# Triton-AI/Triton-Racer-Sim

Hardware: AMD Instinct MI355X
Metric: env-steps/s (whole node) at N envs x 120x160 RGB (higher is better)
Workload: dtype f32 state / f64 nearest-point / u8 image; 1 GPU; 1024 envs/GPU x 1 GPU, bicycle physics + L1 nearest point + 120x160 RGB pinhole rasteriser = BASELINE configs[2], generated_track 1185 pts, synthetic controls seed 0x5EED, auto-reset; envs_total=1024, envs_per_gpu=1024, img_h=120, img_w=160, depth=False, steps_per_launch=1, step_mode=resident worker (posted steps), prewarm_steps=8400, launcher=self

## Files before the change

### triton-racer-sim_amd/csrc/trsim_device.hpp

```cpp
#pragma once
#include <hip/hip_runtime.h>

#include <cstdint>

#include "../../include/trsim.h"
#include "../../include/trsim_spec.h"
#include "trsim_plan.hpp"
#include "trsim_tables.hpp"

#ifndef TRS_ABLATE
#define TRS_ABLATE 0
#endif

namespace trsim {

struct PParams {
    float *x, *y, *z, *yaw, *v, *speed, *cte, *ep_return, *last_return, *steer_filt;
    int32_t *seg_idx, *ep_len;
    uint8_t *done, *pending;
    const float *ctl_steer, *ctl_thr, *ctl_brk;
    const uint8_t* ctl_reset;
    int ctl_stride;
    float4* cam;
    const unsigned char* blob;
// ... 403 lines not shown
    o.is_done = is_done; o.do_reset = do_reset;
}

template <bool SEL = false>
__device__ __forceinline__ void env_step(const PParams& p, const unsigned char* lphys, int e, EnvRegs& s, uint32_t t, int k,
                                         float4* cam_out, float4* lcam_slot, int* pprog_j, int lane, const trsim::HillBlock* hill = nullptr, float* lpitch_slot = nullptr)
{
    const uint8_t rin = (!p.synth && p.ctl_reset && k == 0) ? p.ctl_reset[e] : (uint8_t)0;
    float steer = 0.f, thr = 0.f, brk = 0.f;
    if (!p.synth) {
        const size_t ci = (size_t)k * (size_t)p.ctl_stride + (size_t)e;
        steer = p.ctl_steer[ci]; thr = p.ctl_thr[ci]; brk = p.ctl_brk ? p.ctl_brk[ci] : 0.0f;
    }
    StepOut o;
    env_advance<false, true, SEL>(p, lphys, e, s, t, p.synth, steer, thr, brk, rin, lane, o, hill);
    if (lane == 0) {
        if (p.write_cam) cam_out[e] = o.cam;
        *lcam_slot = o.cam;
        if (hill) {
            if (p.write_cam) hill->cam_pitch[(size_t)(t & (kRing - 1)) * p.n_envs + e] = o.pitch;
            if (lpitch_slot) *lpitch_slot = o.pitch;
        }
        if (o.is_done) atomicAdd(&p.stats[0], 1ull);
        if (o.do_reset) atomicAdd(&p.stats[1], 1ull);
        __hip_atomic_store(pprog_j, k + 1, __ATOMIC_RELEASE, __HIP_MEMORY_SCOPE_WORKGROUP);
    }
}

__device__ __forceinline__ f2v ray_step(f2v kk2, f2v cns)
{
#ifdef TRS_PACKED_RAY_STEP
    return kk2 * cns;
#else
    float dx, dz;
    asm("v_mul_f32 %0, %1, %2" : "=v"(dx) : "v"(kk2.x), "v"(cns.x));
    asm("v_mul_f32 %0, %1, %2" : "=v"(dz) : "v"(kk2.y), "v"(cns.y));
    return f2v{dx, dz};
#endif
}

struct RasterThread {
    const f2v* lrow;
    const float* lrowdepth;
    unsigned pal_off;
    f2v ufa, ufb, ufc, ufd;
    unsigned gwm1, ghm1, pitch;
    int cg, vstart, vground, col_off, row_bytes;
};

__device__ __forceinline__ RasterThread raster_thread(const RParams& p, const unsigned char* lds, int tid)
{
    RasterThread t;
    t.lrow = reinterpret_cast<const f2v*>(lds + p.off_rowtab);
    t.lrowdepth = reinterpret_cast<const float*>(lds + p.off_depth);
    t.pal_off = (unsigned)p.off_pal;
    const float half_w = (float)(p.W / 2);
    t.gwm1 = (unsigned)(p.map_w - 1); t.ghm1 = (unsigned)(p.map_h - 1);
    t.cg = tid % p.gpr;
    const int r0 = tid / p.gpr;
    const float uf0 = (float)(t.cg << 2) + 0.5f - half_w;
    t.ufa = f2v{uf0, uf0}; t.ufb = f2v{uf0 + 1.0f, uf0 + 1.0f}; t.ufc = f2v{uf0 + 2.0f, uf0 + 2.0f}; t.ufd = f2v{uf0 + 3.0f, uf0 + 3.0f};
    t.pitch = (unsigned)p.map_pitch_b;
    t.vstart = r0 < p.rows_per_pass ? r0 : p.H;
    t.vground = t.vstart;
    while (t.vground < p.uni_rows) t.vground += p.rows_per_pass;
    t.row_bytes = p.gpr * 12;
    t.col_off = t.cg * 12;
    return t;
}

struct FrameDesc { __amdgpu_buffer_rsrc_t rgb, dep; };

template <bool DEPTH>
__device__ __forceinline__ FrameDesc frame_desc(const RParams& p, uint8_t* img, float* dep, int e)
{
    FrameDesc f;
    f.rgb = __builtin_amdgcn_make_buffer_rsrc(img + (size_t)e * ((size_t)p.gpe * 12), 0, (int)((size_t)p.gpe * 12), 0x00020000);
    f.dep = f.rgb;
    if constexpr (DEPTH) f.dep = __builtin_amdgcn_make_buffer_rsrc(dep + (size_t)e * ((size_t)p.gpe * 4), 0, (int)((size_t)p.gpe * 16), 0x00020000);
    return f;
}

template <bool DEPTH>
__device__ __forceinline__ void raster_uniform_rows(const RParams& p, const RasterThread& t, const FrameDesc& f, int uni_rows = -1)
{
    const int nu = uni_rows < 0 ? p.uni_rows : uni_rows;
    for (int v = t.vstart; v < nu; v += p.rows_per_pass) {
        const uint32_t c = *(lds_u32p)(uintptr_t)(t.pal_off + ((unsigned)v << 4));
        const u3v px3 = {__builtin_amdgcn_perm(c, c, 0x04020100u), __builtin_amdgcn_perm(c, c, 0x05040201u), __builtin_amdgcn_perm(c, c, 0x06050402u)};
        __builtin_amdgcn_raw_buffer_store_b96(px3, f.rgb, t.col_off + v * t.row_bytes, 0, TRS_STORE_AUX);
        if constexpr (DEPTH) {
            const unsigned dz = __float_as_uint(t.lrowdepth[v]);
            const u4v d4 = {dz, dz, dz, dz};
            __builtin_amdgcn_raw_buffer_store_b128(d4, f.dep, (t.cg + v * p.gpr) * 16, 0, TRS_STORE_AUX);
        }
    }
}

template <bool DEPTH, bool UNI_CHECK = false>
__device__ __forceinline__ void raster_ground_rows(const RParams& p, const RasterThread& t, const FrameDesc& f, const float4 cam)
{
    const f2v sc = {cam.z, cam.w}, cns = {cam.w, -cam.z}, camxz = {cam.x, cam.y};
    f2v rt = t.lrow[t.vground < p.H ? t.vground : 0];
    for (int v = t.vground; v < p.H; v += p.rows_per_pass) {
        const int vn = v + p.rows_per_pass;
        const f2v rtn = t.lrow[vn < p.H ? vn : v];
        const unsigned pal_a = t.pal_off + ((unsigned)v << 4);
        const f2v lz2 = {rt.x, rt.x}, kk2 = {rt.y, rt.y};
        f2v a;
        if constexpr (UNI_CHECK) {
            a.x = __builtin_fmaf(rt.x, sc.x, camxz.x);
            a.y = __builtin_fmaf(rt.x, sc.y, camxz.y);
        } else {
            a = __builtin_elementwise_fma(lz2, sc, camxz);
        }
        const f2v d = ray_step(kk2, cns);
        auto shade = [&](f2v uf) -> uint32_t {
            const f2v g = __builtin_elementwise_fma(uf, d, a);
            const unsigned ix = min(cvt_u32_sat(g.x), t.gwm1);
            const unsigned iz = min(cvt_u32_sat(g.y), t.ghm1);
            const unsigned xoff = (ix >> 2) & ~3u;
            unsigned waddr, paddr;
            asm("v_mad_u32_u24 %0, %1, %2, %3" : "=v"(waddr) : "v"(iz), "s"(t.pitch), "v"(xoff));
            const uint32_t w = *(lds_u32p)(uintptr_t)waddr;
            const uint32_t cls = __builtin_amdgcn_ubfe(w, ix << 1, 2);
            asm("v_lshl_add_u32 %0, %1, 2, %2" : "=v"(paddr) : "v"(cls), "v"(pal_a));
            return *(lds_u32p)(uintptr_t)paddr;
        };
#if TRS_ABLATE == 2
        const uint32_t c0p = (uint32_t)v, c1p = c0p + 1, c2p = c0p + 2, c3p = c0p + 3; (void)shade;
#else
        uint32_t c0p, c1p, c2p, c3p;
        if (UNI_CHECK && rt.y == 0.0f) c0p = c1p = c2p = c3p = *(lds_u32p)(uintptr_t)pal_a;
        else { c0p = shade(t.ufa); c1p = shade(t.ufb); c2p = shade(t.ufc); c3p = shade(t.ufd); }
#endif
        const uint32_t w0 = __builtin_amdgcn_perm(c1p, c0p, 0x04020100u);
        const uint32_t w1 = __builtin_amdgcn_perm(c2p, c1p, 0x05040201u);
        const uint32_t w2 = __builtin_amdgcn_perm(c3p, c2p, 0x06050402u);
#if TRS_ABLATE == 1
        asm volatile("" :: "v"(w0), "v"(w1), "v"(w2)); (void)f;
#else
        const u3v px3 = {w0, w1, w2};
        __builtin_amdgcn_raw_buffer_store_b96(px3, f.rgb, t.col_off + v * t.row_bytes, 0, TRS_STORE_AUX);
        if constexpr (DEPTH) {
            const unsigned dz = __float_as_uint(t.lrowdepth[v]);
            const u4v d4 = {dz, dz, dz, dz};
            __builtin_amdgcn_raw_buffer_store_b128(d4, f.dep, (t.cg + v * p.gpr) * 16, 0, TRS_STORE_AUX);
        }
#endif
        rt = rtn;
    }
}


__device__ __forceinline__ uint32_t hill_filter_colour(const trsim::HillBlock& hb, uint32_t bgr)
{
    int t[3];
#pragma unroll
    for (int ch = 0; ch < 3; ++ch) {
        float x = (float)((bgr >> (8 * ch)) & 255u);
        x = x - hb.f_offset;
        x = x * hb.f_contrast;
        x = x + hb.f_offset;
        x = x < 0.0f ? 0.0f : (x > 255.0f ? 255.0f : x);
        t[ch] = (int)x;
    }
    int o0 = t[0], o1 = t[1], o2 = t[2];
    if (hb.f_color) {
        const int r = t[0], g = t[1], b = t[2];
        const int vv = max(r, max(g, b)), vmin = min(r, min(g, b)), diff = vv - vmin;
        const int sat = (diff * hb.hsv_tab[vv] + (1 << 11)) >> 12;
        int h = (vv == r) ? (g - b) : ((vv == g) ? (b - r + 2 * diff) : (r - g + 4 * diff));
        h = (h * hb.hsv_tab[256 + diff] + (1 << 11)) >> 12;
        if (h < 0) h += 180;
        const int hh = min(h, 255), ss = min(sat, 255);
#pragma unroll
        for (int f = 0; f < 4; ++f) {
            if (f >= hb.f_nfilters) break;
            const int lo = (int)hb.f_lo[f], hi = (int)hb.f_hi[f];
            const bool in = hh >= (lo & 255) && hh <= (hi & 255) && ss >= ((lo >> 8) & 255) && ss <= ((hi >> 8) & 255) && vv >= ((lo >> 16) & 255) && vv <= ((hi >> 16) & 255);
            const int val = in ? 255 : 0, d = hb.f_dst[f];
            o0 = d == 0 ? val : o0; o1 = d == 1 ? val : o1; o2 = d == 2 ? val : o2;
        }
    }
    return (uint32_t)o0 | ((uint32_t)o1 << 8) | ((uint32_t)o2 << 16);
}

__device__ __forceinline__ float hill_row_build(const RParams& p, unsigned char* lds, unsigned tab_off, float P, int v, const float* lg = nullptr)
{
    const trsim::HillBlock hb = *hill_block(p);
    float sp, cp;
    spec_sincos(P, sp, cp);
    const float yn = (hb.hh - ((float)v + 0.5f)) * hb.inv_f;
    const float dy = yn * cp - sp, dz = yn * sp + cp;
    float lz = 0.0f, kk = 0.0f, dep = hb.z_far_f;
    uint32_t c0, c1, c2, c3;
    if (dy >= -1e-6f) {
        c0 = c1 = c2 = c3 = *(lds_u32p)(uintptr_t)((unsigned)hb.off_sky + ((unsigned)v << 2));
        if (lg) { c0 = trsim::light_colour(c0, lg); if (hb.filt) c0 = hill_filter_colour(hb, c0); c1 = c2 = c3 = c0; }
    } else {
        const float t = hb.cam_h_f / (-dy);
        const float zd = t * dz;
        if (zd > hb.z_far_f) {
            c0 = c1 = c2 = c3 = hb.far_rgb;
            if (lg) { c0 = trsim::light_colour(c0, lg); if (hb.filt) c0 = hill_filter_colour(hb, c0); c1 = c2 = c3 = c0; }
        } else {
            lz = zd * hb.inv_cell_f; kk = (t * hb.inv_f) * hb.inv_cell_f; dep = zd;
            const float fw = hb.fog_f * (zd * hb.inv_zfar_f), om = 1.0f - fw;
            constexpr int base[4][3] = {TRS_RGB_GRASS, TRS_RGB_ROAD, TRS_RGB_EDGE, TRS_RGB_CENTRE};
            constexpr int fog[3] = TRS_RGB_FOG;
            uint32_t col[4];
#pragma unroll
            for (int c = 0; c < 4; ++c) {
                uint32_t rgb = 0;
#pragma unroll
                for (int ch = 0; ch < 3; ++ch) {
                    const float a = (float)base[c][ch] * om, b = (float)fog[ch] * fw;
                    const float sum = a + b;
                    rgb |= (uint32_t)(int)(sum + 0.5f) << (8 * ch);
                }
                if (lg) rgb = trsim::light_colour(rgb, lg);
                col[c] = hb.filt ? hill_filter_colour(hb, rgb) : rgb;
            }
            c0 = col[0]; c1 = col[1]; c2 = col[2]; c3 = col[3];
        }
    }
    unsigned char* const tab = lds + tab_off;
    reinterpret_cast<f2v*>(tab)[v] = f2v{lz, kk};
    reinterpret_cast<u4v*>(tab + trsim::hill_table_pal_off(p.H))[v] = u4v{c0, c1, c2, c3};
    reinterpret_cast<float*>(tab + trsim::hill_table_depth_off(p.H))[v] = dep;
    return kk;
}

__device__ __forceinline__ RasterThread raster_use_table(const RasterThread& t, const unsigned char* lds, unsigned tab_off, int H)
{
    RasterThread r = t;
    r.lrow = reinterpret_cast<const f2v*>(lds + tab_off);
    r.pal_off = tab_off + (unsigned)trsim::hill_table_pal_off(H);
    r.lrowdepth = reinterpret_cast<const float*>(lds + tab_off + (unsigned)trsim::hill_table_depth_off(H));
    return r;
}

template <typename Bail>
__device__ __forceinline__ bool team_barrier_wait(const int* dbar, int target, Bail& bail)
{
    for (unsigned spins = 0; __hip_atomic_load(dbar, __ATOMIC_ACQUIRE, __HIP_MEMORY_SCOPE_WORKGROUP) < target; ++spins) {
        __builtin_amdgcn_s_sleep(1);
        if ((spins & 1023u) == 1023u && bail(spins == 1023u)) return false;
    }
    return true;
}

template <typename Bail>
__device__ __forceinline__ bool hill_batch_build(const RParams& p, unsigned char* lds, unsigned tab0, const float (&P)[kHillBatchMax], int nb, int* hbar, int done_before,
                                                 int tid, int lane, Bail& bail, const float* lg0 = nullptr)
{
    constexpr int nrw = kRasterThreads / 64;
    int* const fg = hbar + 4 + 4 * ((done_before / (2 * nrw)) & 1);
    if (tid < kHillBatchMax) fg[tid] = p.H;
    asm volatile("s_waitcnt lgkmcnt(0)" ::: "memory");
    if (lane == 0) __hip_atomic_fetch_add(hbar, 1, __ATOMIC_RELEASE, __HIP_MEMORY_SCOPE_WORKGROUP);
    if (!team_barrier_wait(hbar, done_before + nrw, bail)) return false;
    const unsigned tb = (unsigned)hill_table_bytes(p.H);
    for (int row = tid; row < nb * p.H; row += kRasterThreads) {
        const int bi = row / p.H, v = row - bi * p.H;
        const float Pv = bi == 0 ? P[0] : (bi == 1 ? P[1] : (bi == 2 ? P[2] : P[3]));
        if (hill_row_build(p, lds, tab0 + (unsigned)bi * tb, Pv, v, lg0 ? lg0 + 8 * bi : nullptr) != 0.0f) __hip_atomic_fetch_min(&fg[bi], v, __ATOMIC_RELAXED, __HIP_MEMORY_SCOPE_WORKGROUP);
    }
    asm volatile("s_waitcnt lgkmcnt(0)" ::: "memory");
    if (lane == 0) __hip_atomic_fetch_add(hbar, 1, __ATOMIC_RELEASE, __HIP_MEMORY_SCOPE_WORKGROUP);
    return team_barrier_wait(hbar, done_before + 2 * nrw, bail);
}

template <bool DEPTH>
__device__ __forceinline__ void raster_hill_frame(const RParams& p, const RasterThread& rth, const unsigned char* lds, unsigned tab0, int bi, const int* hbar, int done_before,
                                                  const FrameDesc& f, const float4 cam)
{
    constexpr int nrw = kRasterThreads / 64;
    const int first_ground = hbar[4 + 4 * ((done_before / (2 * nrw)) & 1) + bi];
    RasterThread t = raster_use_table(rth, lds, tab0 + (unsigned)(bi * hill_table_bytes(p.H)), p.H);
    raster_uniform_rows<DEPTH>(p, t, f, first_ground);
    int vg = t.vstart;
    if (vg < first_ground) vg += ((first_ground - vg + p.rows_per_pass - 1) / p.rows_per_pass) * p.rows_per_pass;
    t.vground = vg;
    raster_ground_rows<DEPTH, true>(p, t, f, cam);
}

__device__ __forceinline__ unsigned light_wave_palette(const RParams& p, unsigned pal0, const float* lg, int filt, int wave, int lane)
{
    const unsigned dst = pal0 + (unsigned)((wave % light_copies(p.gpr)) * p.H * 16);
    const int lo = (64 * wave) / p.gpr, hi = min((64 * wave + 63) / p.gpr, p.rows_per_pass - 1);
    const trsim::HillBlock& hb = *hill_block(p);
    float gb[8];
#pragma unroll
    for (int k = 0; k < 8; ++k) gb[k] = lg[k];
    asm volatile("" ::: "memory");
    for (int r0 = lo; r0 <= hi; ++r0)
        for (int i = lane; r0 + (i >> 2) * p.rows_per_pass < p.H; i += 64) {
            const unsigned ent = ((unsigned)(r0 + (i >> 2) * p.rows_per_pass) << 4) + ((unsigned)(i & 3) << 2);
            uint32_t c = trsim::light_colour(*(lds_u32p)(uintptr_t)((unsigned)p.off_pal + ent), gb);
            if (filt) c = hill_filter_colour(hb, c);
            *(__attribute__((address_space(3))) uint32_t*)(uintptr_t)(dst + ent) = c;
        }
    asm volatile("" ::: "memory");
    return dst;
}
// ... 451 lines not shown
```

### triton-racer-sim_amd/csrc/trsim_resident.hip

```cpp
#include <hip/hip_runtime.h>

#include <algorithm>
#include <array>
#include <atomic>
#include <chrono>
#include <cstdint>
#include <cstdlib>
#include <cstring>
#include <mutex>
#include <string>
#include <utility>

#include "../../include/trsim.h"
#include "../../include/trsim_spec.h"
#include "trsim_device.hpp"
#include "trsim_env.hpp"
#include "trsim_internal.hpp"
#include "trsim_post.hpp"

namespace trsim {

struct DevCtl {
    alignas(64) unsigned long long word;
    alignas(64) WEntry ring[kSlots];
// ... 330 lines not shown
        }
    }
}

template <bool DEPTH, bool DYN, bool HILLS = false, bool LENS = false, bool LIGHT = false>
__global__ __launch_bounds__(kBlock) void trs_worker_kernel(const WParams wp)
{
    const int tid = threadIdx.x, lane = tid & 63, wave = tid >> 6;
    const bool raster_team = tid < kRasterThreads;
    const RParams& p = wp.ra;
    const PParams& P = wp.ph;
    const int epw = p.envs_per_wg;
    const WLds l = wlds_of(smem + wp.lds_off_ctl, epw);
    const int e_begin = blockIdx.x * epw;
    const int n_loc = min(e_begin + epw, p.n_envs) - e_begin;
    const int pw = wave - kRasterThreads / 64;
    if ((unsigned)(uintptr_t)smem != 0u) {
        if (tid == 0) {
            atomicAdd(&p.stats[2], 1ull);
            sys_store64(p.fault, 1ull);
            sys_store64(&wp.mb->error, ((u64)kGiveUpLdsBase << 32) | (u64)blockIdx.x);
            __hip_atomic_fetch_or(&wp.dc->word, kAbortBit, __ATOMIC_RELAXED, __HIP_MEMORY_SCOPE_AGENT);
            if (blockIdx.x == 0) { sys_store64(&wp.mb->consumed, wp.start); sys_store64(&wp.mb->exited, 1ull); }
        }
        return;
    }
    if (raster_team) stage_lds_dma(p.blob, p.blob_bytes, 0u, wave, kRasterThreads / 64, lane);
    else stage_lds_dma(P.blob, P.blob_bytes, (unsigned)wp.lds_off_phys, pw, kPhysWaves, lane);
    if (LENS && raster_team) lens_stage_palette(p, (unsigned)wp.lds_off_hill, wave, lane);
    if (tid == 0) { lds_store64(l.word, wp.start); lds_store64(l.fwd, wp.start); }
    if (tid < kSlots) l.arrive[tid] = 0;
    for (int j = tid; j < 2 * epw; j += kBlock) l.pprog[j] = 0;
    int* const hbar = reinterpret_cast<int*>(smem + wp.lds_off_hill + hill_batch(p.H) * hill_table_bytes(p.H));
    if (HILLS && tid == 0) *hbar = 0;
    const int lds_off_light = worker_lds_light(wp.lds_off_hill, p.H, variant_bits(DEPTH, DYN, HILLS, LENS, LIGHT));
    float* const lring = reinterpret_cast<float*>(smem + lds_off_light);
    const unsigned lds_off_lpal = (unsigned)lds_off_light + (unsigned)(kCamDepth * epw * 32);
    const float* const light_g = LIGHT ? hill_block(p)->light : nullptr;
    const int lfilt = LIGHT ? hill_block(p)->filt : 0;
    if constexpr (DYN) {
        if (tid < 32) reinterpret_cast<int*>(smem + wp.fp.lds_off + kDynBatch * p.H * 16)[tid] = 0;
        dyn_stage_tables(smem, wp.fp, p.H, tid, kBlock, reinterpret_cast<const uint32_t*>(p.blob + p.off_pal));
    }
    if (!raster_team)
        for (int j = pw; j < n_loc; j += kPhysWaves) {
            EnvRegs st;
            env_load(P, e_begin + j, st);
            const float lr = coherent_load(&P.last_return[e_begin + j]);
            if (lane == 0) {
                float* q = l.lst + (size_t)j * 16;
                q[0] = st.x; q[1] = st.y; q[2] = st.z; q[3] = st.yaw; q[4] = st.v; q[5] = st.sf; q[6] = st.epr;
                q[7] = __int_as_float(st.seg); q[8] = __int_as_float(st.epl); q[9] = __int_as_float(st.done); q[10] = __int_as_float(st.pend);
                q[11] = lr;
            }
        }
    asm volatile("s_waitcnt vmcnt(0) lgkmcnt(0)" ::: "memory");
    __syncthreads();
    if (tid == 0) worker_checkin(wp);

    if (!raster_team) {
        const int first = blockIdx.x == 0 ? 1 : 0, nphys = kPhysWaves - first;
        if (pw < first) { dispatcher_run(wp, l, lane); return; }
        Duties D{blockIdx.x != 0 && pw == 0, pw == kPhysWaves - 1, wp.start};
        if (D.leader && !leader_wait_decision(wp, l, lane)) return;
        const unsigned char* const lphys = smem + wp.lds_off_phys;
        u64 s = wp.start;
        for (;; ++s) {
            const int r = (int)(s - wp.start);
            if (!wait_posted(wp, l, D, s, lane)) break;
            const u64* en = reinterpret_cast<const u64*>(&wp.dc->ring[s & (kSlots - 1)]);
            const u64 ev = lane < 6 ? agent_load64(en + lane) : 0ull;
            const float* const c_st = reinterpret_cast<const float*>(lane_u64(ev, 1));
            const float* const c_th = reinterpret_cast<const float*>(lane_u64(ev, 2));
            const float* const c_br = reinterpret_cast<const float*>(lane_u64(ev, 3));
            const uint8_t* const c_rs = reinterpret_cast<const uint8_t*>(lane_u64(ev, 4));
            const int synth = (int)(unsigned)lane_u64(ev, 5);
            for (int j = pw - first; j < n_loc; j += nphys) {
                const int e = e_begin + j;
                if (r >= kCamDepth && !wait_lds_ge(wp, l, &D, &l.rread[j], (r - kCamDepth + 1) * (kRasterThreads / 64), kGiveUpCamRing, lane)) return;
                float steer = 0.f, thr = 0.f, brk = 0.f;
                uint8_t rin = 0;
                if (!synth) {
                    steer = sys_load_val(&c_st[e]); thr = sys_load_val(&c_th[e]);
                    if (c_br) brk = sys_load_val(&c_br[e]);
                    if (c_rs) rin = sys_load_val(&c_rs[e]);
                }
                float* const q = l.lst + (size_t)j * 16;
                EnvRegs st;
                st.x = q[0]; st.y = q[1]; st.z = q[2]; st.yaw = q[3]; st.v = q[4]; st.sf = q[5]; st.epr = q[6];
                st.seg = __float_as_int(q[7]); st.epl = __float_as_int(q[8]); st.done = __float_as_int(q[9]); st.pend = __float_as_int(q[10]);
                st.speed = 0.f; st.cte = 0.f;
                float lr = q[11];
                const float epr_before = st.epr;
                StepOut o;
                if (n_loc <= TRS_PHYS_PRIO_MAX_ENVS) __builtin_amdgcn_s_setprio(3);
                env_advance<true, false>(P, lphys, e, st, (uint32_t)s, synth, steer, thr, brk, rin, lane, o, HILLS ? hill_block(p) : nullptr);
                if (n_loc <= TRS_PHYS_PRIO_MAX_ENVS) __builtin_amdgcn_s_setprio(0);
                if (o.do_reset) lr = epr_before;
                if constexpr (LIGHT) {
                    const float lv = lane < 8 ? sys_load_val(&light_g[(size_t)e * 8 + lane]) : 0.f;
                    if (lane < 8) lring[((size_t)(r & (kCamDepth - 1)) * epw + j) * 8 + lane] = lv;
                }
                if (lane == 0) {
                    q[0] = st.x; q[1] = st.y; q[2] = st.z; q[3] = st.yaw; q[4] = st.v; q[5] = st.sf; q[6] = st.epr;
                    q[7] = __int_as_float(st.seg); q[8] = __int_as_float(st.epl); q[9] = __int_as_float(st.done); q[10] = __int_as_float(st.pend);
                    q[11] = lr;
                    float* const sl = l.slot + ((size_t)(r & (kCamDepth - 1)) * epw + j) * kSlotWords;
                    *reinterpret_cast<float4*>(sl) = o.cam;
                    sl[4] = st.x; sl[5] = st.y; sl[6] = st.z; sl[7] = st.yaw; sl[8] = st.v; sl[9] = st.speed; sl[10] = st.cte;
                    sl[11] = __int_as_float(st.seg); sl[12] = st.epr; sl[13] = __int_as_float(st.epl); sl[14] = st.sf; sl[15] = lr;
                    sl[16] = __int_as_float(st.done);
                    if constexpr (HILLS) sl[17] = o.pitch;
                    if (o.is_done) atomicAdd(&P.stats[0], 1ull);
                    if (o.do_reset) atomicAdd(&P.stats[1], 1ull);
                    drain_lds();
                    lds_store32(&l.pprog[j], r + 1);
                }
            }
        }
        if (D.forwarder) {
            u64 t0 = 0;
            for (unsigned spins = 0; D.fwd < s; ++spins) {
                forward_arrivals(wp, l, D.fwd, lane);
                if (lds_load64(l.word) & kAbortBit) break;
                __builtin_amdgcn_s_sleep(2);
                if ((spins & 1023u) == 1023u) {
                    const u64 now = (u64)wall_clock64();
                    if (t0 == 0) t0 = now;
                    else if (now - t0 > wp.safety_ticks) { worker_abort(wp, l, kGiveUpForward); break; }
                }
            }
        }
        return;
    }

    const RasterThread rth = raster_thread(p, smem, tid);
    trsim::LensBlock lb{};
    LensCacheWorker<DEPTH> lcache;
    if constexpr (LENS) {
        lb = *lens_block(p);
        lens_cache_load(p, rth, lb, lcache);
    }
    int nu = 0, ng = 0;
    for (int v = rth.vstart; v < p.uni_rows; v += p.rows_per_pass) ++nu;
    for (int v = rth.vground; v < p.H; v += p.rows_per_pass) ++ng;
#pragma unroll
    for (int off = 32; off >= 1; off >>= 1) { nu = max(nu, __shfl_xor(nu, off, 64)); ng = max(ng, __shfl_xor(ng, off, 64)); }
    nu *= DEPTH ? 2 : 1; ng *= DEPTH ? 2 : 1;
    int own = 0;
    for (int j = wave; j < n_loc; j += kRasterThreads / 64) ++own;
    const int nuni = nu * n_loc, nstep = (nu + ng) * n_loc + 2 * own;
    constexpr bool kSkipUniform = !DYN && !HILLS && !LIGHT && !LENS;
    const int lag = worker_lag(nstep, nuni, kSkipUniform);
    unsigned char* optr = nullptr;
    {
        unsigned char* const tab[14] = {(unsigned char*)P.x, (unsigned char*)P.y, (unsigned char*)P.z, (unsigned char*)P.yaw, (unsigned char*)P.v,
                                        (unsigned char*)P.speed, (unsigned char*)P.cte, (unsigned char*)P.seg_idx, (unsigned char*)P.ep_return,
                                        (unsigned char*)P.ep_len, (unsigned char*)P.steer_filt, (unsigned char*)P.last_return,
                                        (unsigned char*)P.done, (unsigned char*)P.pending};
#pragma unroll
        for (int k = 0; k < 14; ++k) optr = lane == k ? tab[k] : optr;
    }
    Duties none{false, false, 0};
    u64 owed = wp.start;
    const bool probe = (kDiag & 4) && blockIdx.x == 7 && wave == 0;
    auto now_clk = [&]() -> u64 { u64 t; asm volatile("s_memtime %0\n\ts_waitcnt lgkmcnt(0)" : "=s"(t) :: "memory"); return t; };
    u64 t_post = 0, t_pose = 0, t_vm = 0, t_all = 0, t_mark = probe ? now_clk() : 0;
    for (u64 s = wp.start;; ++s) {
        const int r = (int)(s - wp.start);
        if (owed < s && (lds_load64(l.word) & kCountMask) <= s) {
            drain_vmem();
            for (; owed < s; ++owed) raster_arrive(l, owed, lane);
        }
        const u64 tp0 = probe ? now_clk() : 0;
        if (!wait_posted(wp, l, none, s, lane)) {
            drain_vmem();
            for (; owed < s; ++owed) raster_arrive(l, owed, lane);
            if (probe && lane == 0) {
                t_all = now_clk() - t_mark;
                atomicAdd(&p.stats[40], t_post); atomicAdd(&p.stats[41], t_pose); atomicAdd(&p.stats[42], t_vm); atomicAdd(&p.stats[43], t_all);
                atomicAdd(&p.stats[44], (u64)r);
            }
            return;
        }
        if (probe) t_post += now_clk() - tp0;
        uint8_t* const img = (s & 1ull) ? wp.img1 : wp.img0;
        float* const dep = (s & 1ull) ? wp.dep1 : wp.dep0;
        const u64 ahead = (lds_load64(l.word) & kCountMask) - 1 - s;
        const u64 keep = ahead + 1 < (u64)lag ? ahead + 1 : (u64)lag;
        if constexpr (DYN) {
            while (s - owed >= keep) {
                wait_vmcnt_le((int)(s - owed - 1) * nstep);
                raster_arrive(l, owed++, lane);
            }
            const int nbatch = (n_loc + kDynBatch - 1) / kDynBatch;
            for (int b0 = 0; b0 < n_loc; b0 += kDynBatch) {
                float4 cams[kDynBatch];
                unsigned tel = 0; int mine_j = -1;
#pragma unroll
                for (int bi = 0; bi < kDynBatch; ++bi) {
                    const int j = b0 + bi;
                    cams[bi] = make_float4(0.f, 0.f, 0.f, 1.f);
                    if (j < n_loc) {
                        if (!wait_lds_ge(wp, l, nullptr, &l.pprog[j], r + 1, kGiveUpPhysics, lane)) return;
                        const float* const sl = l.slot + ((size_t)(r & (kCamDepth - 1)) * epw + j) * kSlotWords;
                        cams[bi] = *reinterpret_cast<const float4*>(sl);
                        if ((j % (kRasterThreads / 64)) == wave) { mine_j = j; tel = __float_as_uint(sl[4 + min(lane, 12)]); }
                        asm volatile("s_waitcnt lgkmcnt(0)" :: "v"(cams[bi].x), "v"(cams[bi].y), "v"(cams[bi].z), "v"(cams[bi].w), "v"(tel) : "memory");
                        if (!LIGHT && lane == 0) __hip_atomic_fetch_add(&l.rread[j], 1, __ATOMIC_RELAXED, __HIP_MEMORY_SCOPE_WORKGROUP);
                    }
                }
                u64 t0_bar = 0;
                auto bail = [&](bool first) -> bool {
                    if (lds_load64(l.word) & kAbortBit) return true;
                    const u64 now = (u64)wall_clock64();
                    if (first) { t0_bar = now; return false; }
                    if (now - t0_bar > wp.safety_ticks) { worker_abort(wp, l, kGiveUpBarrier); return true; }
                    return false;
                };
                if (!raster_dyn_batch<DEPTH, LIGHT>(p, wp.fp, rth, smem, cams, min(kDynBatch, n_loc - b0), img, dep, e_begin + b0, r * nbatch + b0 / kDynBatch, tid, lane, bail,
                                                   LIGHT ? lring + ((size_t)(r & (kCamDepth - 1)) * epw + b0) * 8 : nullptr, lds_off_lpal)) return;
                if (LIGHT && lane == 0)
                    for (int bi = 0; bi < kDynBatch && b0 + bi < n_loc; ++bi) __hip_atomic_fetch_add(&l.rread[b0 + bi], 1, __ATOMIC_RELAXED, __HIP_MEMORY_SCOPE_WORKGROUP);
                if (mine_j >= 0 && !(kDiag & 2)) {
                    const size_t e = (size_t)(e_begin + mine_j);
                    if (lane < 12) __hip_atomic_store((__attribute__((address_space(1))) unsigned*)(uintptr_t)optr + e, tel, __ATOMIC_RELAXED, __HIP_MEMORY_SCOPE_SYSTEM);
                    else if (lane < 14) __hip_atomic_store((__attribute__((address_space(1))) unsigned char*)(uintptr_t)optr + e, (unsigned char)(lane == 12 ? tel : 0u), __ATOMIC_RELAXED, __HIP_MEMORY_SCOPE_SYSTEM);
                }
            }
            continue;
        }
        if constexpr (HILLS) {
            while (s - owed >= keep) {
                wait_vmcnt_le((int)(s - owed - 1) * nstep);
                raster_arrive(l, owed++, lane);
            }
            const int HB = hill_batch(p.H);
            const int nbatch = (n_loc + HB - 1) / HB;
            for (int b0 = 0; b0 < n_loc; b0 += HB) {
                const int nb = min(HB, n_loc - b0);
                float4 cams[kHillBatchMax]; float Pv[kHillBatchMax];
                unsigned tel = 0; int mine_j = -1;
#pragma unroll
                for (int bi = 0; bi < kHillBatchMax; ++bi) {
                    cams[bi] = make_float4(0.f, 0.f, 0.f, 1.f); Pv[bi] = 0.f;
                    const int j = b0 + bi;
                    if (bi < nb) {
                        if (!wait_lds_ge(wp, l, nullptr, &l.pprog[j], r + 1, kGiveUpPhysics, lane)) return;
                        const float* const sl = l.slot + ((size_t)(r & (kCamDepth - 1)) * epw + j) * kSlotWords;
                        cams[bi] = *reinterpret_cast<const float4*>(sl);
                        Pv[bi] = sl[17];
                        if ((j % (kRasterThreads / 64)) == wave) { mine_j = j; tel = __float_as_uint(sl[4 + min(lane, 12)]); }
                        asm volatile("s_waitcnt lgkmcnt(0)" :: "v"(cams[bi].x), "v"(cams[bi].y), "v"(cams[bi].z), "v"(cams[bi].w), "v"(tel), "v"(Pv[bi]) : "memory");
                        if (!LIGHT && lane == 0) __hip_atomic_fetch_add(&l.rread[j], 1, __ATOMIC_RELAXED, __HIP_MEMORY_SCOPE_WORKGROUP);
                    }
                }
                u64 t0_bar = 0;
                auto bail = [&](bool first) -> bool {
                    if (lds_load64(l.word) & kAbortBit) return true;
                    const u64 now = (u64)wall_clock64();
                    if (first) { t0_bar = now; return false; }
                    if (now - t0_bar > wp.safety_ticks) { worker_abort(wp, l, kGiveUpBarrier); return true; }
                    return false;
                };
                const int done_before = (r * nbatch + b0 / HB) * 2 * (kRasterThreads / 64);
                if (!hill_batch_build(p, smem, (unsigned)wp.lds_off_hill, Pv, nb, hbar, done_before, tid, lane, bail,
                                      LIGHT ? lring + ((size_t)(r & (kCamDepth - 1)) * epw + b0) * 8 : nullptr)) return;
                if (LIGHT && lane == 0)
                    for (int bi = 0; bi < nb; ++bi) __hip_atomic_fetch_add(&l.rread[b0 + bi], 1, __ATOMIC_RELAXED, __HIP_MEMORY_SCOPE_WORKGROUP);
#pragma unroll
                for (int bi = 0; bi < kHillBatchMax; ++bi)
                    if (bi < nb)
                        raster_hill_frame<DEPTH>(p, rth, smem, (unsigned)wp.lds_off_hill, bi, hbar, done_before, frame_desc<DEPTH>(p, img, dep, e_begin + b0 + bi), cams[bi]);
                if (mine_j >= 0 && !(kDiag & 2)) {
                    const size_t e = (size_t)(e_begin + mine_j);
                    if (lane < 12) __hip_atomic_store((__attribute__((address_space(1))) unsigned*)(uintptr_t)optr + e, tel, __ATOMIC_RELAXED, __HIP_MEMORY_SCOPE_SYSTEM);
                    else if (lane < 14) __hip_atomic_store((__attribute__((address_space(1))) unsigned char*)(uintptr_t)optr + e, (unsigned char)(lane == 12 ? tel : 0u), __ATOMIC_RELAXED, __HIP_MEMORY_SCOPE_SYSTEM);
                }
            }
            continue;
        }
        if constexpr (LIGHT && !HILLS && !DYN) {
            for (int j = 0; j < n_loc; ++j) {
                const FrameDesc fd = frame_desc<DEPTH>(p, img, dep, e_begin + j);
                if (!wait_lds_ge(wp, l, nullptr, &l.pprog[j], r + 1, kGiveUpPhysics, lane)) return;
                const float* const sl = l.slot + ((size_t)(r & (kCamDepth - 1)) * epw + j) * kSlotWords;
                const float4 cam = *reinterpret_cast<const float4*>(sl);
                const bool mine = (j % (kRasterThreads / 64)) == wave;
                unsigned tel = 0;
                if (mine) tel = __float_as_uint(sl[4 + min(lane, 12)]);
                RasterThread rl = rth;
                rl.pal_off = light_wave_palette(p, lds_off_lpal, lring + ((size_t)(r & (kCamDepth - 1)) * epw + j) * 8, lfilt, wave, lane);
                asm volatile("s_waitcnt lgkmcnt(0)" :: "v"(cam.x), "v"(cam.y), "v"(cam.z), "v"(cam.w), "v"(tel) : "memory");
                if (lane == 0) __hip_atomic_fetch_add(&l.rread[j], 1, __ATOMIC_RELAXED, __HIP_MEMORY_SCOPE_WORKGROUP);
                raster_uniform_rows<DEPTH>(p, rl, fd);
                if (j == 0)
                    while (s - owed >= keep) {
                        wait_vmcnt_le((int)(s - owed - 1) * nstep + nu);
                        raster_arrive(l, owed++, lane);
                    }
                raster_ground_rows<DEPTH>(p, rl, fd, cam);
                if (mine && !(kDiag & 2)) {
                    const size_t e = (size_t)(e_begin + j);
                    if (lane < 12) __hip_atomic_store((__attribute__((address_space(1))) unsigned*)(uintptr_t)optr + e, tel, __ATOMIC_RELAXED, __HIP_MEMORY_SCOPE_SYSTEM);
                    else if (lane < 14) __hip_atomic_store((__attribute__((address_space(1))) unsigned char*)(uintptr_t)optr + e, (unsigned char)(lane == 12 ? tel : 0u), __ATOMIC_RELAXED, __HIP_MEMORY_SCOPE_SYSTEM);
                }
            }
            continue;
        }
        const bool skipu = kSkipUniform && worker_skips_uniform(wp.uni_mask, wp.start, s);
        const bool sweep = ahead == 0 && !skipu;
        if (sweep)
            for (int j = 0; j < n_loc; ++j) raster_uniform_rows<DEPTH>(p, rth, frame_desc<DEPTH>(p, img, dep, e_begin + j));
        for (int j = 0; j < n_loc; ++j) {
            const FrameDesc fd = frame_desc<DEPTH>(p, img, dep, e_begin + j);
            if (!sweep && !skipu) raster_uniform_rows<DEPTH>(p, rth, fd);
            if (j == 0)
                while (s - owed >= keep) {
                    const u64 tv0 = probe ? now_clk() : 0;
                    if (!(kDiag & 1))
                        wait_vmcnt_le(kSkipUniform ? worker_wait_count(wp.uni_mask, wp.start, owed, s, nstep, nuni, skipu ? 0 : (sweep ? nuni : nu))
                                                   : (int)(s - owed - 1) * nstep + (sweep ? nuni : nu));
                    if (probe) t_vm += now_clk() - tv0;
                    raster_arrive(l, owed++, lane);
                }
            const u64 tq0 = probe ? now_clk() : 0;
            if (!wait_lds_ge(wp, l, nullptr, &l.pprog[j], r + 1, kGiveUpPhysics, lane)) return;
            if (probe) t_pose += now_clk() - tq0;
            const float* const sl = l.slot + ((size_t)(r & (kCamDepth - 1)) * epw + j) * kSlotWords;
            const float4 cam = *reinterpret_cast<const float4*>(sl);
            const bool mine = (j % (kRasterThreads / 64)) == wave;
            unsigned tel = 0;
            if (mine) tel = __float_as_uint(sl[4 + min(lane, 12)]);
            asm volatile("s_waitcnt lgkmcnt(0)" :: "v"(cam.x), "v"(cam.y), "v"(cam.z), "v"(cam.w), "v"(tel) : "memory");
            if (lane == 0) __hip_atomic_fetch_add(&l.rread[j], 1, __ATOMIC_RELAXED, __HIP_MEMORY_SCOPE_WORKGROUP);
            if constexpr (LENS) raster_lens_frame(p, rth, lb, lcache, (unsigned)wp.lds_off_hill, fd, cam);
            else raster_ground_rows<DEPTH>(p, rth, fd, cam);
            if (mine && !(kDiag & 2)) {
                const size_t e = (size_t)(e_begin + j);
                if (lane < 12) __hip_atomic_store((__attribute__((address_space(1))) unsigned*)(uintptr_t)optr + e, tel, __ATOMIC_RELAXED, __HIP_MEMORY_SCOPE_SYSTEM);
                else if (lane < 14) __hip_atomic_store((__attribute__((address_space(1))) unsigned char*)(uintptr_t)optr + e, (unsigned char)(lane == 12 ? tel : 0u), __ATOMIC_RELAXED, __HIP_MEMORY_SCOPE_SYSTEM);
            }
        }
    }
}

using WorkerKernel = void (*)(WParams);
template <Variant V> WorkerKernel worker_kernel_of()
{
    if constexpr (variant_built(V)) return &trs_worker_kernel<(V & kVDepth) != 0, (V & kVDyn) != 0, (V & kVHills) != 0, (V & kVLens) != 0, (V & kVLight) != 0>;
    else return nullptr;
}
template <Variant... V> std::array<WorkerKernel, kVariants> worker_kernel_table(std::integer_sequence<Variant, V...>) { return {worker_kernel_of<V>()...}; }
const std::array<WorkerKernel, kVariants> kWorkerKernels = worker_kernel_table(std::make_integer_sequence<Variant, kVariants>{});

constexpr int kPwEnvs = 4;
constexpr int kPwBlock = 64 * (kPwEnvs + 2);

__global__ __launch_bounds__(kPwBlock) void trs_physics_worker_kernel(const WParams wp)
{
    const int tid = threadIdx.x, lane = tid & 63, wave = tid >> 6;
    const PParams& P = wp.ph;
    const WLds l = wlds_of(smem + wp.lds_off_ctl, kPwEnvs);
    const int e_begin = blockIdx.x * kPwEnvs;
    const int n_loc = min(e_begin + kPwEnvs, P.n_envs) - e_begin;
    if ((unsigned)(uintptr_t)smem != 0u) {
        if (tid == 0) {
            atomicAdd(&P.stats[2], 1ull);
            sys_store64(P.fault, 1ull);
            sys_store64(&wp.mb->error, ((u64)kGiveUpLdsBase << 32) | (u64)blockIdx.x);
            __hip_atomic_fetch_or(&wp.dc->word, kAbortBit, __ATOMIC_RELAXED, __HIP_MEMORY_SCOPE_AGENT);
            if (blockIdx.x == 0) { sys_store64(&wp.mb->consumed, wp.start); sys_store64(&wp.mb->exited, 1ull); }
        }
        return;
    }
    stage_lds_dma(P.blob, P.blob_bytes, 0u, wave, kPwBlock / 64, lane);
    if (tid == 0) { lds_store64(l.word, wp.start); lds_store64(l.fwd, wp.start); }
    if (tid < kSlots) l.arrive[tid] = 0;
    asm volatile("s_waitcnt vmcnt(0) lgkmcnt(0)" ::: "memory");
    __syncthreads();
    if (tid == 0) worker_checkin(wp);

    if (wave == kPwEnvs + 1) {
        if (blockIdx.x == 0) dispatcher_run(wp, l, lane);
        return;
    }
    if (wave == kPwEnvs) {
        Duties D{blockIdx.x != 0, true, wp.start, n_loc};
        if (D.leader && !leader_wait_decision(wp, l, lane)) return;
        u64 s = wp.start;
        while (wait_posted(wp, l, D, s, lane)) ++s;
        const u64 w = lds_load64(l.word);
        if (w & kAbortBit) return;
        const u64 last = w & kCountMask;
        u64 t0 = 0;
        for (unsigned spins = 0; D.fwd < last; ++spins) {
            forward_arrivals(wp, l, D.fwd, lane, n_loc);
            if (lds_load64(l.word) & kAbortBit) break;
            __builtin_amdgcn_s_sleep(2);
            if ((spins & 1023u) == 1023u) {
                const u64 now = (u64)wall_clock64();
                if (t0 == 0) t0 = now;
                else if (now - t0 > wp.safety_ticks) { worker_abort(wp, l, kGiveUpForward); break; }
            }
        }
        return;
    }
    if (wave >= n_loc) return;

    const int e = e_begin + wave;
    EnvRegs st;
    env_load(P, e, st);
    float lr = coherent_load(&P.last_return[e]);
    unsigned char* optr = nullptr;
    {
        unsigned char* const tab[14] = {(unsigned char*)P.x, (unsigned char*)P.y, (unsigned char*)P.z, (unsigned char*)P.yaw, (unsigned char*)P.v,
                                        (unsigned char*)P.speed, (unsigned char*)P.cte, (unsigned char*)P.seg_idx, (unsigned char*)P.ep_return,
                                        (unsigned char*)P.ep_len, (unsigned char*)P.steer_filt, (unsigned char*)P.last_return,
                                        (unsigned char*)P.done, (unsigned char*)P.pending};
#pragma unroll
        for (int k = 0; k < 14; ++k) optr = lane == k ? tab[k] : optr;
    }
    Duties none{false, false, 0};
    u64 owed = wp.start;
    struct Ctl { float steer, thr, brk; uint8_t rin; int synth; };
    auto entry_load = [&](u64 s) -> u64 {
        const u64* en = reinterpret_cast<const u64*>(&wp.dc->ring[s & (kSlots - 1)]);
        return lane < 6 ? agent_load64(en + lane) : 0ull;
    };
    auto ctl_load = [&](u64 ev) -> Ctl {
        const float* const c_st = reinterpret_cast<const float*>(lane_u64(ev, 1));
        const float* const c_th = reinterpret_cast<const float*>(lane_u64(ev, 2));
        const float* const c_br = reinterpret_cast<const float*>(lane_u64(ev, 3));
        const uint8_t* const c_rs = reinterpret_cast<const uint8_t*>(lane_u64(ev, 4));
        Ctl in{0.f, 0.f, 0.f, 0, (int)(unsigned)lane_u64(ev, 5)};
        asm volatile("" :: "s"(c_st), "s"(c_th), "s"(in.synth) : "memory");
        if (!in.synth) {
            in.steer = sys_load_val(&c_st[e]); in.thr = sys_load_val(&c_th[e]);
            if (c_br) in.brk = sys_load_val(&c_br[e]);
            if (c_rs) in.rin = sys_load_val(&c_rs[e]);
        }
        return in;
    };
    bool have_ctl = false, have_ent = false;
    Ctl nxt{};
    u64 ent_next = 0ull;
    u64 clean_below = wp.start;
    for (u64 s = wp.start;; ++s) {
        if (owed < s && (lds_load64(l.word) & kCountMask) <= s) {
            drain_vmem();
            for (; owed < s; ++owed) raster_arrive(l, owed, lane);
            clean_below = s;
        }
        Ctl in;
        if (have_ctl) {
            in = nxt;
        } else {
            if (!wait_posted(wp, l, none, s, lane)) {
                drain_vmem();
                for (; owed < s; ++owed) raster_arrive(l, owed, lane);
                return;
            }
            in = ctl_load(entry_load(s));
            drain_vmem();
            clean_below = s;
        }
        const u64 count = lds_load64(l.word) & kCountMask;
        have_ctl = count > s + 1;
        if (have_ctl) {
            const bool was_prefetched = have_ent;
            nxt = ctl_load(was_prefetched ? ent_next : entry_load(s + 1));
            const u64 c = was_prefetched ? s - 1 : s;
            clean_below = c > clean_below ? c : clean_below;
        }
        have_ent = have_ctl && count > s + 2;
        if (have_ent) ent_next = entry_load(s + 2);
        for (; owed < clean_below; ++owed) raster_arrive(l, owed, lane);
        const float epr_before = st.epr;
        StepOut o;
        env_advance<true, false, true>(P, smem, e, st, (uint32_t)s, in.synth, in.steer, in.thr, in.brk, in.rin, lane, o);
        if (o.do_reset) lr = epr_before;
        if (lane == 0) {
            if (o.is_done) atomicAdd(&P.stats[0], 1ull);
            if (o.do_reset) atomicAdd(&P.stats[1], 1ull);
        }
        unsigned tel = 0;
        {
            const unsigned vals[13] = {__float_as_uint(st.x), __float_as_uint(st.y), __float_as_uint(st.z), __float_as_uint(st.yaw), __float_as_uint(st.v),
                                       __float_as_uint(st.speed), __float_as_uint(st.cte), (unsigned)st.seg, __float_as_uint(st.epr), (unsigned)st.epl,
                                       __float_as_uint(st.sf), __float_as_uint(lr), (unsigned)st.done};
// ... 404 lines not shown
```

Baseline: 125.3 million env-steps/s.

## Software-pipeline ground-row raster across three LDS/store stages

Adds a three-stage software-pipelined version of the ground-row rasteriser for the non-depth path. It overlaps map-texel LDS reads, palette LDS reads, and buffer stores across consecutive row trips, using explicit lgkmcnt waits and scheduling barriers. The trip count is made wave-uniform once per worker. The aim is to hide LDS latency between dependent lookups. In exchange it uses more registers for the two in-flight stages and relies on hand-tuned waitcnt encodings, with clamped addresses and a guarded store at the tail.

```diff
diff --git a/triton-racer-sim_amd/csrc/trsim_device.hpp b/triton-racer-sim_amd/csrc/trsim_device.hpp
--- a/triton-racer-sim_amd/csrc/trsim_device.hpp
+++ b/triton-racer-sim_amd/csrc/trsim_device.hpp
@@ -579,6 +579,95 @@
     }
 }
 
+struct MapReads { uint32_t w0, w1, w2, w3; unsigned s0, s1, s2, s3; };
+struct PalReads { uint32_t c0, c1, c2, c3; };
+
+__device__ __forceinline__ int ground_row_trips(const RParams& p, const RasterThread& t)
+{
+    int n = t.vground < p.H ? (p.H - 1 - t.vground) / p.rows_per_pass + 1 : 0;
+#pragma unroll
+    for (int off = 32; off >= 1; off >>= 1) n = max(n, __shfl_xor(n, off, 64));
+    return __builtin_amdgcn_readfirstlane(n);
+}
+
+__device__ __forceinline__ void raster_ground_rows_pipelined(const RParams& p, const RasterThread& t, const FrameDesc& f, const float4 cam, const int ntrip)
+{
+#if TRS_ABLATE != 0
+    (void)ntrip;
+    raster_ground_rows<false>(p, t, f, cam);
+#else
+    if (t.vground >= p.H) return;
+    const f2v sc = {cam.z, cam.w}, cns = {cam.w, -cam.z}, camxz = {cam.x, cam.y};
+    const int vlast = p.H - 1, rpp = p.rows_per_pass;
+    constexpr int kLater = 9;
+    constexpr int kWaitLater = 0xC07F | (kLater << 8), kWaitEntry = 0xC07F | ((kLater - 1) << 8);
+    typedef __attribute__((address_space(3))) const f2v* lds_f2vp;
+    const unsigned ra_last = (unsigned)p.off_rowtab + ((unsigned)vlast << 3), pa_last = t.pal_off + ((unsigned)vlast << 4);
+    const unsigned frame_bytes = (unsigned)(p.H * t.row_bytes);
+    unsigned ra = (unsigned)p.off_rowtab + ((unsigned)t.vground << 3);
+    unsigned pa = t.pal_off + ((unsigned)(t.vground - rpp) << 4);
+    unsigned so = (unsigned)(t.col_off + (t.vground - 2 * rpp) * t.row_bytes);
+    auto next_trip = [&]() { pa += (unsigned)rpp << 4; so += (unsigned)(rpp * t.row_bytes); };
+    auto stage1 = [&](f2v& rt, MapReads& m) {
+        __builtin_amdgcn_s_waitcnt(kWaitEntry); __builtin_amdgcn_sched_barrier(0);
+        const f2v lz2 = {rt.x, rt.x}, kk2 = {rt.y, rt.y};
+        const f2v a = __builtin_elementwise_fma(lz2, sc, camxz);
+        const f2v d = ray_step(kk2, cns);
+        ra = min(ra + ((unsigned)rpp << 3), ra_last);
+        rt = *(lds_f2vp)(uintptr_t)ra;
+        __builtin_amdgcn_sched_barrier(0);
+        auto look = [&](f2v uf, uint32_t& w, unsigned& sh) {
+            const f2v g = __builtin_elementwise_fma(uf, d, a);
+            const unsigned ix = min(cvt_u32_sat(g.x), t.gwm1);
+            const unsigned iz = min(cvt_u32_sat(g.y), t.ghm1);
+            const unsigned xoff = (ix >> 2) & ~3u;
+            unsigned waddr;
+            asm("v_mad_u32_u24 %0, %1, %2, %3" : "=v"(waddr) : "v"(iz), "s"(t.pitch), "v"(xoff));
+            w = *(lds_u32p)(uintptr_t)waddr;
+            sh = ix << 1;
+        };
+        look(t.ufa, m.w0, m.s0); look(t.ufb, m.w1, m.s1); look(t.ufc, m.w2, m.s2); look(t.ufd, m.w3, m.s3);
+        __builtin_amdgcn_sched_barrier(0);
+    };
+    auto stage2 = [&](const MapReads& m, PalReads& c, bool last) {
+        __builtin_amdgcn_s_waitcnt(kWaitLater); __builtin_amdgcn_sched_barrier(0);
+        const unsigned pal_a = last ? min(pa, pa_last) : pa;
+        auto colour = [&](uint32_t w, unsigned sh) -> uint32_t {
+            const uint32_t cls = __builtin_amdgcn_ubfe(w, sh, 2);
+            unsigned paddr;
+            asm("v_lshl_add_u32 %0, %1, 2, %2" : "=v"(paddr) : "v"(cls), "v"(pal_a));
+            return *(lds_u32p)(uintptr_t)paddr;
+        };
+        c.c0 = colour(m.w0, m.s0); c.c1 = colour(m.w1, m.s1); c.c2 = colour(m.w2, m.s2); c.c3 = colour(m.w3, m.s3);
+        __builtin_amdgcn_sched_barrier(0);
+    };
+    auto stage3 = [&](const PalReads& c, bool last) {
+        __builtin_amdgcn_s_waitcnt(kWaitLater); __builtin_amdgcn_sched_barrier(0);
+        const u3v px3 = {__builtin_amdgcn_perm(c.c1, c.c0, 0x04020100u), __builtin_amdgcn_perm(c.c2, c.c1, 0x05040201u), __builtin_amdgcn_perm(c.c3, c.c2, 0x06050402u)};
+        if (!last || so < frame_bytes) __builtin_amdgcn_raw_buffer_store_b96(px3, f.rgb, (int)so, 0, TRS_STORE_AUX);
+    };
+    MapReads ma, mb;
+    PalReads ca, cb;
+    f2v rt = *(lds_f2vp)(uintptr_t)ra;
+    stage1(rt, ma); next_trip();
+    if (ntrip == 1) { stage2(ma, ca, true); next_trip(); stage3(ca, true); return; }
+    stage1(rt, mb); stage2(ma, ca, false); next_trip();
+    int k = 2;
+    for (; k + 1 < ntrip; k += 2) {
+        stage1(rt, ma); stage2(mb, cb, false); stage3(ca, false); next_trip();
+        stage1(rt, mb); stage2(ma, ca, false); stage3(cb, false); next_trip();
+    }
+    if (k < ntrip) {
+        stage1(rt, ma); stage2(mb, cb, false); stage3(ca, false); next_trip();
+        stage2(ma, ca, true); stage3(cb, false); next_trip();
+        stage3(ca, true);
+    } else {
+        stage2(mb, cb, true); stage3(ca, false); next_trip();
+        stage3(cb, true);
+    }
+#endif
+}
+
 
 __device__ __forceinline__ uint32_t hill_filter_colour(const trsim::HillBlock& hb, uint32_t bgr)
 {
diff --git a/triton-racer-sim_amd/csrc/trsim_resident.hip b/triton-racer-sim_amd/csrc/trsim_resident.hip
--- a/triton-racer-sim_amd/csrc/trsim_resident.hip
+++ b/triton-racer-sim_amd/csrc/trsim_resident.hip
@@ -506,6 +506,8 @@
     const int nuni = nu * n_loc, nstep = (nu + ng) * n_loc + 2 * own;
     constexpr bool kSkipUniform = !DYN && !HILLS && !LIGHT && !LENS;
     const int lag = worker_lag(nstep, nuni, kSkipUniform);
+    [[maybe_unused]] int gtrips = 0;
+    if constexpr (kSkipUniform && !DEPTH) gtrips = ground_row_trips(p, rth);
     unsigned char* optr = nullptr;
     {
         unsigned char* const tab[14] = {(unsigned char*)P.x, (unsigned char*)P.y, (unsigned char*)P.z, (unsigned char*)P.yaw, (unsigned char*)P.v,
@@ -689,7 +691,8 @@
             asm volatile("s_waitcnt lgkmcnt(0)" :: "v"(cam.x), "v"(cam.y), "v"(cam.z), "v"(cam.w), "v"(tel) : "memory");
             if (lane == 0) __hip_atomic_fetch_add(&l.rread[j], 1, __ATOMIC_RELAXED, __HIP_MEMORY_SCOPE_WORKGROUP);
             if constexpr (LENS) raster_lens_frame(p, rth, lb, lcache, (unsigned)wp.lds_off_hill, fd, cam);
-            else raster_ground_rows<DEPTH>(p, rth, fd, cam);
+            else if constexpr (DEPTH) raster_ground_rows<DEPTH>(p, rth, fd, cam);
+            else raster_ground_rows_pipelined(p, rth, fd, cam, gtrips);
             if (mine && !(kDiag & 2)) {
                 const size_t e = (size_t)(e_begin + j);
                 if (lane < 12) __hip_atomic_store((__attribute__((address_space(1))) unsigned*)(uintptr_t)optr + e, tel, __ATOMIC_RELAXED, __HIP_MEMORY_SCOPE_SYSTEM);
```

New measurement: 129.4 million env-steps/s (median of 6 runs). 3.3% higher.
